# natir/br

Hardware: AMD Instinct MI355X
Metric: corrected Gbases/sec at k=19, 10 kb ONT-error reads (higher is better)
Workload: dtype u64 k-mers / 1-bit set

## Files before the change

### br_amd/csrc/brx_onelane.hip

```cpp
#include "brx_correct.hpp"

#include <stdlib.h>
#include <algorithm>
#include <vector>

using namespace brx;

namespace brx {
uint64_t scan_tmp_bytes(uint32_t n);
int exclusive_scan_lens(const uint32_t *d_lens, uint32_t n, uint64_t *d_tmp, uint64_t *d_out_offsets,
                        unsigned long long *d_total, hipStream_t s);
}


namespace {

constexpr uint32_t U_VOID = 0xffffffffu;
constexpr uint32_t U_END = 0xffffffffu;
constexpr uint32_t C_FAIL = 0xfffffff1u;
constexpr uint32_t C_VOID = 0xfffffff2u;
constexpr uint32_t U_UNWRITTEN = 0xffffffffu;
constexpr int MAX_DEPTH = 3;
constexpr uint32_t MAX_LANE_READ = 1u << 28;
#ifndef BRX_AP_EDITS
// ... 75 lines not shown
    __builtin_memcpy(&q, in + (n - 16u - j), 16);
    return make_uint4(__builtin_bswap32(q.w), __builtin_bswap32(q.z), __builtin_bswap32(q.y), __builtin_bswap32(q.x));
}
__device__ __forceinline__ uint4 ld16_raw(const uint8_t *in, uint32_t n, uint32_t j, bool flip)
{
    uint4 q;
    __builtin_memcpy(&q, in + (flip ? n - 16u - j : j), 16);
    return q;
}
__device__ __forceinline__ uint4 ld16_turn(const uint4 &q, bool flip)
{
    return flip ? make_uint4(__builtin_bswap32(q.w), __builtin_bswap32(q.z), __builtin_bswap32(q.y), __builtin_bswap32(q.x)) : q;
}
__device__ __forceinline__ uint64_t pack_start(uint64_t in_at, uint32_t r) { return (in_at >> 4) + 5ull * r; }
__device__ __forceinline__ uint64_t edit_start(uint64_t in_at, uint32_t r, uint64_t ub, uint32_t jj, uint32_t q)
{
    return (in_at >> 2) + 16ull * (ub + r + jj) + (uint64_t)(q >> 2);
}

__global__ __launch_bounds__(256) void lane_units_kernel(LaneArgs a)
{
    const uint32_t r = blockIdx.x * 256u + threadIdx.x;
    if (r >= a.p.n_reads)
        return;
    const uint8_t *in;
    uint32_t n;
    bool poisoned;
    (void)read_view(a.p, r, in, n, poisoned);
    const uint32_t C = chunk_of(a, r);
    a.nu[r] = n < 2u * C ? 1u : n / C;
}

__global__ __launch_bounds__(256) void lane_pack_kernel(LaneArgs a)
{
    for (uint32_t r = blockIdx.x; r < a.p.n_reads; r += gridDim.x) {
        const uint8_t *in;
        uint32_t n;
        bool poisoned;
        const uint64_t at = read_view(a.p, r, in, n, poisoned);
        uint32_t *dst = a.P + pack_start(at, r);
        const uint32_t ndw = (n >> 4) + 5u;
        for (uint32_t d = threadIdx.x; d < ndw; d += 256) {
            const uint32_t b = 16u * d;
            uint32_t w[4] = {0, 0, 0, 0};
            if (b + 16u <= n) {
                const uint4 q = ld16_logical(in, n, b, a.p.flip);
                w[0] = q.x;
                w[1] = q.y;
                w[2] = q.z;
                w[3] = q.w;
            } else {
                for (uint32_t t = 0; t < 16u && b + t < n; t++)
                    w[t >> 2] |= (uint32_t)ld_logical(in, n, b + t, a.p.flip) << (8u * (t & 3u));
            }
            uint32_t v = 0;
#pragma unroll
            for (int t = 0; t < 4; t++)
                v = (v << 8) | ((((w[t] >> 1) & 0x03030303u) * 0x40100401u) >> 24);
            dst[d] = v;
        }
        const uint64_t ub = a.ubase[r], ue = a.ubase[r + 1];
        for (uint64_t u = ub + threadIdx.x; u < ue; u += 256) {
            a.u_read[u] = r;
            a.u_in[u] = make_uint4((uint32_t)at, (uint32_t)(at >> 32), n, (uint32_t)(u - ub));
        }
    }
}

template <bool IDX>
__device__ __forceinline__ bool set_get(const PassParams &p, uint64_t km, int k)
{
    if (!IDX)
        return probe(p.bits, km, k);
    uint64_t key;
    const uint32_t home = index_locate(p.idx, km, k, key);
    for (uint32_t hop = 0;; hop++) {
        const int pr = index_probe_at(p.idx, key, home, hop);
        if (pr != 2)
            return pr == 1;
        if (p.bits) {
            const uint64_t h = key - 1ull;
            return (p.bits[h >> 5] >> (h & 31u)) & 1u;
        }
    }
}

template <bool IDX>
__global__ __launch_bounds__(256) void lane_mask_kernel(LaneArgs a)
{
    const PassParams &p = a.p;
    const int lane = threadIdx.x & 63;
    const int k = p.k;
    const uint64_t mask = kmask(k);
    const unsigned long long n_units = p.ctrl[CTL_LANE_UNITS];
    const unsigned long long wave = (unsigned long long)blockIdx.x * 4ull + (threadIdx.x >> 6);
    const unsigned long long n_waves = (unsigned long long)gridDim.x * 4ull;
    const bool filter = p.idx.line_bits != nullptr && p.idx.line_shift >= 6u;
    uint4 ui_next = wave < n_units ? a.u_in[wave] : make_uint4(0, 0, 0, 0);
    uint32_t r_next = wave < n_units ? a.u_read[wave] : 0u;
    for (unsigned long long u = wave; u < n_units; u += n_waves) {
        const uint4 ui = ui_next;
        const uint32_t r = r_next;
        if (u + n_waves < n_units) {
            ui_next = a.u_in[u + n_waves];
            r_next = a.u_read[u + n_waves];
        }
        const uint32_t j = ui.w, n = ui.z;
        const uint64_t at = ((uint64_t)ui.y << 32) | ui.x;
        const bool last = (uint64_t)j + 1ull == a.ubase[r + 1] - a.ubase[r];
        const uint32_t C = chunk_of(a, r);
        const uint32_t s = (j * C) & ~15u;
        const uint32_t lim = last ? n : ((j + 1u) * C) & ~15u;
        const uint32_t *row = a.P + pack_start(at, r);
        uint16_t *mrow = a.M + pack_start(at, r);
        uint64_t carry = 0;
        if (s) {
            const uint32_t b = s - 31u, w = b >> 4, sh = 2u * (b & 15u);
            const uint64_t hi = ((uint64_t)row[w] << 32) | row[w + 1];
            const uint64_t lo = row[w + 2];
            carry = (sh ? ((hi << sh) | (lo >> (32u - sh))) : hi) >> 2;
        }
        for (uint32_t e0 = s; e0 < lim; e0 += 64u) {
            const uint32_t e = e0 + (uint32_t)lane;
            const uint32_t code = (row[e >> 4] >> (30u - 2u * (e & 15u))) & 3u;
            const uint64_t km = lane_kmer64_dpp(carry, code, lane, mask);
            bool sol = false;
            if (e < lim && e + 1u >= (uint32_t)k) {
                if (IDX) {
                    uint64_t key;
                    const uint32_t home = index_locate(p.idx, km, k, key);
                    if (!filter || ((p.idx.line_bits[home >> 5] >> (home & 31u)) & 1u)) {
                        int pr = index_probe_at(p.idx, key, home, 0u);
                        for (uint32_t hop = 1; pr == 2 && !p.bits; hop++)
                            pr = index_probe_at(p.idx, key, home, hop);
                        if (pr == 2) {
                            const uint64_t h = key - 1ull;
                            pr = (p.bits[h >> 5] >> (h & 31u)) & 1u;
                        }
                        sol = pr == 1;
                    }
                } else {
                    sol = probe(p.bits, km, k);
                }
            }
            const uint64_t ball = __ballot(sol);
            if ((lane & 15) == 0 && e < lim)
                mrow[e >> 4] = (uint16_t)(ball >> lane);
            carry = ((uint64_t)(uint32_t)__builtin_amdgcn_readlane((int)(uint32_t)(km >> 32), 63) << 32) |
                    (uint32_t)__builtin_amdgcn_readlane((int)(uint32_t)km, 63);
        }
    }
}

template <bool IDX>
__global__ __launch_bounds__(256) void lane_sync_kernel(LaneArgs a)
{
    const PassParams &p = a.p;
    const uint32_t lane = threadIdx.x & 63u, half = lane >> 5, hl = lane & 31u;
    const uint32_t k = (uint32_t)p.k;
    const unsigned long long n_units = p.ctrl[CTL_LANE_UNITS];
    const unsigned long long wave = (unsigned long long)blockIdx.x * 4ull + (threadIdx.x >> 6);
    const unsigned long long n_waves = (unsigned long long)gridDim.x * 4ull;
    for (unsigned long long u0 = 2ull * wave; u0 < n_units; u0 += 2ull * n_waves) {
        const unsigned long long u = u0 + half;
        const bool mine = u < n_units;
        const uint4 ui = mine ? a.u_in[u] : make_uint4(0, 0, 0, 0);
        const uint32_t j = ui.w, n = ui.z;
        const uint32_t r = mine ? a.u_read[u] : 0u;
        const uint64_t at = ((uint64_t)ui.y << 32) | ui.x;
        const uint32_t *row = a.P + pack_start(at, r);
        const uint32_t C = chunk_of(a, r);
        const uint32_t s = j * C;
        const uint32_t lim = (s + C < n) ? s + C : n;
        const uint32_t e0 = s + k - 1u;
        bool open_ = mine && j != 0u;
        uint32_t q = (mine && j == 0u) ? 0u : U_VOID;
        uint64_t qk = 0;
        uint32_t prev32 = 0;
        for (uint32_t t = 0; __any(open_ && e0 + 32u * t < lim); t++) {
            const uint32_t e = e0 + 32u * t + hl;
            const bool valid = open_ && e < lim;
            uint64_t km = 0;
            bool sol = false;
            if (valid) {
                const uint32_t b = e + 1u - k, wd = b >> 4, sh = 2u * (b & 15u);
                const uint64_t hi = ((uint64_t)row[wd] << 32) | row[wd + 1];
                const uint64_t lo = row[wd + 2];
                km = (sh ? ((hi << sh) | (lo >> (32u - sh))) : hi) >> (64u - 2u * k);
                sol = set_get<IDX>(p, km, (int)k);
            }
            const uint64_t ball = __ballot(sol);
            const uint32_t cur32 = (uint32_t)(ball >> (32u * half));
            const uint64_t w = ((uint64_t)cur32 << 32) | prev32;
            uint64_t x = w;
            for (uint32_t rr = 1; rr < a.R; rr++)
                x &= w << rr;
            const uint32_t hit = (uint32_t)(x >> 32);
            const bool found = open_ && hit != 0u;
            const uint32_t el_l = found ? (uint32_t)__builtin_ctz(hit) : 0u;
            const uint32_t src = 32u * half + el_l;
            const uint32_t klo = (uint32_t)__shfl((int)(uint32_t)km, (int)src), khi = (uint32_t)__shfl((int)(uint32_t)(km >> 32), (int)src);
            if (found) {
                const uint32_t qq = e0 + 32u * t + el_l + 1u;
                if (qq < n) {
                    q = qq;
                    qk = ((uint64_t)khi << 32) | klo;
                }
                open_ = false;
            } else if (open_ && e0 + 32u * (t + 1u) >= lim) {
                open_ = false;
            }
            prev32 = cur32;
        }
        if (mine && hl == 0u) {
            a.u_q[u] = q;
            if (j != 0u)
                a.u_qk[u] = qk;
        }
    }
}

__global__ __launch_bounds__(256) void lane_sync_mask_kernel(LaneArgs a)
{
    const PassParams &p = a.p;
    const uint32_t k = (uint32_t)p.k;
    const unsigned long long n_units = p.ctrl[CTL_LANE_UNITS];
    for (unsigned long long u = (unsigned long long)blockIdx.x * 256ull + threadIdx.x; u < n_units; u += (unsigned long long)gridDim.x * 256ull) {
        const uint4 ui = a.u_in[u];
        const uint32_t j = ui.w, n = ui.z;
        if (j == 0) {
            a.u_q[u] = 0;
            continue;
        }
        const uint32_t r = a.u_read[u];
        const uint64_t at = ((uint64_t)ui.y << 32) | ui.x;
        const uint32_t *row = a.P + pack_start(at, r);
        const uint16_t *mrow = a.M + pack_start(at, r);
        const uint32_t C = chunk_of(a, r);
        const uint32_t s = j * C;
        const uint32_t lim = (s + C < n) ? s + C : n;
        const uint32_t e0 = s + k - 1u;
        uint32_t q = U_VOID;
        uint64_t qk = 0;
        uint64_t w = 0;
        for (uint32_t g = e0 >> 4; 16u * g < lim; g++) {
            uint32_t bits = mrow[g];
            const uint32_t base = 16u * g;
            if (base < e0)
                bits &= 0xffffu << (e0 - base);
            if (base + 16u > lim)
                bits &= 0xffffu >> (base + 16u - lim);
            w = (w >> 16) | ((uint64_t)bits << 48);
            uint64_t t = w;
            for (uint32_t rr = 1; rr < a.R; rr++)
                t &= w << rr;
            const uint32_t hit = (uint32_t)(t >> 48);
            if (hit) {
                const uint32_t el = base + (uint32_t)__builtin_ctz(hit);
                if (el + 1u < n) {
                    q = el + 1u;
                    const uint32_t b = el + 1u - k, wd = b >> 4, sh = 2u * (b & 15u);
                    const uint64_t hi = ((uint64_t)row[wd] << 32) | row[wd + 1];
                    const uint64_t lo = row[wd + 2];
                    qk = (sh ? ((hi << sh) | (lo >> (32u - sh))) : hi) >> (64u - 2u * k);
                }
                break;
            }
        }
        a.u_q[u] = q;
        a.u_qk[u] = qk;
    }
}

struct __attribute__((aligned(16))) UnitDesc {
    uint32_t n;
    uint32_t q;
    uint32_t t1;
    uint32_t tgt;
    uint64_t tgtk;
    uint64_t eat;
    uint64_t pw;
    uint32_t ecap;
    uint32_t first;
};

__global__ __launch_bounds__(256) void lane_link_kernel(LaneArgs a)
{
    const PassParams &p = a.p;
    const unsigned long long n_units = p.ctrl[CTL_LANE_UNITS];
    for (unsigned long long u = (unsigned long long)blockIdx.x * 256ull + threadIdx.x; u < n_units; u += (unsigned long long)gridDim.x * 256ull) {
        const uint32_t r = a.u_read[u];
        const uint32_t ub = (uint32_t)a.ubase[r], uend = (uint32_t)a.ubase[r + 1];
        const uint8_t *in;
        uint32_t n;
        bool poisoned;
        const uint64_t in_at = read_view(p, r, in, n, poisoned);
        UnitDesc d;
        d.n = n;
        d.q = n >= MAX_LANE_READ ? U_VOID - 1u : a.u_q[u];
        uint32_t t = (uint32_t)u + 1u;
        while (t < uend && a.u_q[t] == U_VOID)
            t++;
        const uint32_t q0 = d.q >= U_VOID - 1u ? 0u : d.q;
        d.eat = edit_start(in_at, r, ub, (uint32_t)u - ub, q0);
        uint64_t end_at;
        if (t < uend) {
            d.t1 = t;
            d.tgt = a.u_q[t];
            d.tgtk = a.u_qk[t];
            end_at = edit_start(in_at, r, ub, t - ub, d.tgt);
        } else {
            d.t1 = U_END;
            d.tgt = n;
            d.tgtk = 0;
            end_at = edit_start(in_at, r, ub, uend - ub, n);
        }
        d.ecap = (uint32_t)(end_at - d.eat);
        d.pw = pack_start(in_at, r) + (q0 >> 4);
        d.first = (uint32_t)u == ub ? 1u : 0u;
        a.u_desc[u] = d;
    }
}

enum { S_ST = 0, S_CUR = 2, S_JJ = 4, S_ACC = 8, S_PASS = 12, S_DIRTY = 16, S_SKIP = 24, S_PREV = 27, S_FIRST = 28, S_SLOW = 29 };
constexpr uint32_t MASK_STEP = 16;

template <bool IDX, int KT, bool MASK>
__global__ __launch_bounds__(256, MASK ? 6 : BRX_LANE_WAVES) void lane_kernel(LaneArgs a)
{
    const PassParams &p = a.p;
    const int k = KT ? KT : p.k;
    const uint32_t c = (uint32_t)p.c;
    const uint64_t mask = kmask(k);
    const unsigned long long n_units = p.ctrl[CTL_LANE_UNITS];
    __shared__ uint4 lc[4][256];
    const uint32_t tid = threadIdx.x;

    bool have = false, want = true;
    uint32_t u = 0, n = 0, i = 0, tgt = 0, t1 = U_END;
    uint64_t tgtk = 0;
    uint32_t depth = 0, ne = 0, ecap = 0;
// ... 1449 lines not shown
    const char *e = getenv(name);
    return e && *e ? (uint32_t)strtoul(e, nullptr, 10) : dflt;
}

void lane_ws_free(brx_chain *ch)
{
    delete (LaneWork *)ch->lane_ws;
    ch->lane_ws = nullptr;
}

int lane_pass(brx_chain *ch, const PassParams &p, const LanePassInfo &info, hipStream_t s)
{
    const bool walk = info.method != BRX_ONE;
    if (env_u32("BRX_LANE", 1u) == 0u || p.k > 31 || p.n_reads == 0)
        return BRX_ERR_UNSUPPORTED;
    if (info.method != BRX_GRAPH && (p.c < 1 || p.c > 5))
        return BRX_ERR_UNSUPPORTED;
    if (walk && env_u32("BRX_LANE_WALK", 1u) == 0u)
        return BRX_ERR_UNSUPPORTED;
    if (!walk && p.idx.lines && 32u - p.idx.line_shift > env_u32("BRX_LANE_MAX_LOG_LINES", 26u))
        return BRX_ERR_UNSUPPORTED;
    const bool idx = p.idx.lines != nullptr;
    if (!idx && !p.bits)
        return BRX_ERR_UNSUPPORTED;
    constexpr uint64_t RESIDENT = 256ull * 4ull * BRX_LANE_WAVES * 64ull;
    uint32_t C = env_u32("BRX_LANE_CHUNK", 0u);
    if (C == 0u) {
        const uint64_t want = info.in_total_bound / (4ull * RESIDENT);
        C = want < 256ull ? 256u : (want > 2048ull ? 2048u : (uint32_t)want);
    }
    if (C < 64u)
        C = 64u;
    uint32_t R = env_u32("BRX_LANE_SYNC", 4u);
    if (R < 1u)
        R = 1u;
    if (R > 32u)
        R = 32u;

    LaneWork *w = (LaneWork *)ch->lane_ws;
    if (!w) {
        w = new LaneWork();
        ch->lane_ws = w;
    }
    const bool graded = !walk && env_u32("BRX_LANE_TAIL", 0u) != 0u && p.n_reads >= 64u;
    const uint32_t r_half = graded ? p.n_reads - p.n_reads / 5u : 0xffffffffu;
    const uint32_t r_quarter = graded ? p.n_reads - p.n_reads / 20u : 0xffffffffu;
    const uint32_t c_min = graded ? ((C >> 2) < 64u ? 64u : (C >> 2)) : C;
    const uint64_t units_bound = info.in_total_bound / c_min + (uint64_t)p.n_reads + 1ull;
    if (units_bound >= 0xfffffff0ull)
        return BRX_ERR_UNSUPPORTED;
    const uint64_t p_bound = (info.in_total_bound >> 4) + 5ull * p.n_reads + 16ull;
    const uint64_t e_bound = (info.in_total_bound >> 2) + 16ull * (units_bound + 2ull * p.n_reads) + 64ull;
    const char *what = "lane pass workspace";
    const uint64_t n = p.n_reads, hr = n / 8 + 64;
    BRX_TRY(w->nu.reserve(n, hr, what));
    BRX_TRY(w->fail_list.reserve(n, hr, what));
    BRX_TRY(w->ubase.reserve(n + 1, hr, what));
    const uint64_t hu = units_bound / 8 + 64;
    BRX_TRY(w->u_read.reserve(units_bound, hu, what));
    BRX_TRY(w->u_q.reserve(units_bound, hu, what));
    BRX_TRY(w->u_qk.reserve(units_bound, hu, what));
    BRX_TRY(w->u_res.reserve(units_bound * 8, hu * 8, what));
    BRX_TRY(w->u_desc.reserve(units_bound, hu, what));
    BRX_TRY(w->u_in.reserve(units_bound, hu, what));
    BRX_TRY(w->P.reserve(p_bound, p_bound / 16, what));
    BRX_TRY(w->M.reserve(p_bound, p_bound / 16, what));
    for (int d = 0; d < MAX_DEPTH; d++)
        BRX_TRY(w->E[d].reserve(e_bound, e_bound / 16, what));
    if (walk)
        for (int d = 0; d < MAX_DEPTH; d++)
            BRX_TRY(w->BW[d].reserve(e_bound, e_bound / 16, what));
    if (scan_tmp_bytes(p.n_reads) > ch->d_scan_tmp.bytes()) {
        set_error("lane pass: scan scratch smaller than the batch");
        return BRX_ERR_ARG;
    }
    LaneArgs a;
    a.p = p;
    a.C = C;
    a.r_half = r_half;
    a.r_quarter = r_quarter;
    a.R = R;
    a.nu = w->nu;
    a.ubase = w->ubase;
    a.u_read = w->u_read;
    a.u_q = w->u_q;
    a.u_qk = w->u_qk;
    a.u_res = w->u_res;
    a.u_desc = w->u_desc;
    a.u_in = w->u_in;
    a.P = w->P;
    const uint32_t mask_mode = env_u32("BRX_LANE_MASK", 1u);
    const bool use_mask = walk ? mask_mode >= 1u : mask_mode >= 2u;
    a.M = use_mask ? w->M : nullptr;
    for (int d = 0; d < MAX_DEPTH; d++) {
        a.E[d] = w->E[d];
        a.EW[d] = reinterpret_cast<uint2 *>(w->E[d].get());
        a.BW[d] = w->BW[d];
    }
    if (info.method == BRX_GRAPH)
        a.p.c = 1;
    a.fail_list = w->fail_list;
    a.succ = nullptr;
    a.dbg = nullptr;
    DevBuf<unsigned long long> d_dbg;
#ifdef BRX_LANE_TIMING
    if (!walk && env_u32("BRX_LANE_TIMING", 0u) != 0u) {
        BRX_TRY(d_dbg.reserve(1 + 3 * 16384, 0, "lane timing"));
        BRX_HIP(hipMemsetAsync(d_dbg, 0, (1 + 3 * 16384) * 8, s));
        a.dbg = d_dbg;
    }
#endif
    if (walk && idx && env_u32("BRX_LANE_SUCC", 1u) != 0u) {
        brx_set *set = const_cast<brx_set *>(ch->set);
        std::lock_guard<std::mutex> g(set->idx_mu);
        const uint64_t n_lines = 1ull << (32u - p.idx.line_shift);
        if (!set->d_succ || set->succ_lines != n_lines || set->succ_gen != set->idx_gen) {
            if (set->succ_lines != n_lines)
                set->d_succ.reset();
            BRX_TRY(set->d_succ.reserve(n_lines, 0, "successor table"));
            set->succ_lines = n_lines;
            KernelTimer t("succ_build", s);
            const uint64_t blocks = (n_lines + 255ull) / 256ull;
            succ_build_kernel<<<(uint32_t)(blocks < 65536ull ? blocks : 65536ull), 256, 0, s>>>(p, n_lines, set->d_succ);
            BRX_HIP(hipGetLastError());
            BRX_HIP(hipStreamSynchronize(s));
            set->succ_gen = set->idx_gen;
        }
        a.succ = set->d_succ;
    }

    const uint32_t rb = (p.n_reads + 255u) / 256u;
    {
        KernelTimer t("lane_units", s);
        BRX_HIP(hipMemsetAsync(p.ctrl + CTL_LANE_UNITS, 0, (CTL_LANE_FAIL + 1 - CTL_LANE_UNITS) * 8, s));
        BRX_HIP(hipMemsetAsync(w->u_res, 0xff, units_bound * 32ull, s));
        lane_units_kernel<<<rb, 256, 0, s>>>(a);
        BRX_TRY(exclusive_scan_lens(w->nu, p.n_reads, ch->d_scan_tmp, w->ubase, p.ctrl + CTL_LANE_UNITS, s));
        const uint32_t grid = read_grid(p.n_reads, 1u << 16);
        lane_pack_kernel<<<grid, 256, 0, s>>>(a);
    }
    if (use_mask) {
        KernelTimer t("lane_mask", s);
        BRX_HIP(hipMemsetAsync(w->M, 0, p_bound * 2ull, s));
        const uint64_t waves = units_bound < 256ull * 32ull ? units_bound : 256ull * 32ull;
        const uint32_t blocks = (uint32_t)((waves + 3) / 4);
        if (idx)
            lane_mask_kernel<true><<<blocks, 256, 0, s>>>(a);
        else
            lane_mask_kernel<false><<<blocks, 256, 0, s>>>(a);
    }
    {
        KernelTimer t("lane_sync", s);
        const uint64_t waves = units_bound < 256ull * 32ull ? units_bound : 256ull * 32ull;
        const uint32_t blocks = (uint32_t)((waves + 3) / 4);
        if (use_mask) {
            const uint64_t ub = (units_bound + 255ull) / 256ull;
            lane_sync_mask_kernel<<<(uint32_t)(ub < 16384ull ? ub : 16384ull), 256, 0, s>>>(a);
        } else if (idx)
            lane_sync_kernel<true><<<blocks, 256, 0, s>>>(a);
        else
            lane_sync_kernel<false><<<blocks, 256, 0, s>>>(a);
        const uint64_t lb = (units_bound + 255ull) / 256ull;
        lane_link_kernel<<<(uint32_t)(lb < 4096ull ? lb : 4096ull), 256, 0, s>>>(a);
    }
    {
        static const char *names[5] = {"correct_pass", "correct_pass_two", "correct_pass_graph", "correct_pass_greedy", "correct_pass_gap_size"};
        KernelTimer t(names[info.method], s);
        const uint64_t want = (units_bound + 255ull) / 256ull;
        const uint64_t waves = walk ? (uint64_t)walk_waves(info.method) : (use_mask ? 6ull : (uint64_t)BRX_LANE_WAVES);
        const uint32_t blocks = (uint32_t)(want < 256ull * waves ? want : 256ull * waves);
        if (info.method == BRX_ONE) {
            if (idx && use_mask)
                launch_lane<true, true>(a, blocks, s);
            else if (idx)
                launch_lane<true, false>(a, blocks, s);
            else if (use_mask)
                launch_lane<false, true>(a, blocks, s);
            else
                launch_lane<false, false>(a, blocks, s);
        } else if (info.method == BRX_GRAPH) {
            if (idx)
                launch_lane_walk<true, BRX_GRAPH>(a, blocks, s);
            else
                launch_lane_walk<false, BRX_GRAPH>(a, blocks, s);
        } else {
            if (idx)
                launch_lane_walk<true, BRX_GAP_SIZE>(a, blocks, s);
            else
                launch_lane_walk<false, BRX_GAP_SIZE>(a, blocks, s);
        }
    }
    if (d_dbg) {
        std::vector<unsigned long long> h(1 + 3 * 16384);
        BRX_HIP(hipMemcpyAsync(h.data(), d_dbg, h.size() * 8, hipMemcpyDeviceToHost, s));
        BRX_HIP(hipStreamSynchronize(s));
        const size_t nw = (size_t)(h[0] < 16384ull ? h[0] : 16384ull);
        if (nw) {
            std::vector<double> st(nw), en(nw), it(nw), lr(nw);
            unsigned long long t0 = ~0ull;
            for (size_t i = 0; i < nw; i++)
                t0 = h[1 + 3 * i] < t0 ? h[1 + 3 * i] : t0;
            for (size_t i = 0; i < nw; i++) {
                st[i] = (double)(h[1 + 3 * i] - t0) * 0.01;
                en[i] = (double)(h[2 + 3 * i] - t0) * 0.01;
                it[i] = (double)(h[3 + 3 * i] & 0xffffffffull);
                lr[i] = (double)(h[3 + 3 * i] >> 32);
            }
            auto pct = [](std::vector<double> v, double q) { std::sort(v.begin(), v.end()); return v[(size_t)(q * (double)(v.size() - 1))]; };
            fprintf(stderr, "[lane timing] %zu waves, %u reads; start us p0/p50/p100 %.0f/%.0f/%.0f; end us p0/p10/p50/p90/p99/p100 %.0f/%.0f/%.0f/%.0f/%.0f/%.0f; "
                            "loop iterations per wave p0/p50/p100 %.0f/%.0f/%.0f; lane-rounds per wave p50/p100 %.0f/%.0f\n",
                    nw, p.n_reads, pct(st, 0), pct(st, .5), pct(st, 1), pct(en, 0), pct(en, .1), pct(en, .5), pct(en, .9), pct(en, .99), pct(en, 1),
                    pct(it, 0), pct(it, .5), pct(it, 1), pct(lr, .5), pct(lr, 1));
        }
    }
    {
        KernelTimer t("lane_apply", s);
        const uint32_t gcap = env_u32("BRX_AP_GRID", 1u << 20);
        const uint32_t grid = p.n_reads < gcap ? p.n_reads : gcap;
        if (walk)
            lane_apply_walk_kernel<<<grid, 256, 0, s>>>(a);
        else
            lane_apply_kernel<<<grid, AP_BS, 0, s>>>(a);
    }
    {
        KernelTimer t("lane_redo", s);
        PassParams q = p;
        q.only = w->fail_list;
        q.only_n = p.ctrl + CTL_LANE_FAIL;
        BRX_HIP(hipMemsetAsync(p.ctrl + CTL_WORK, 0, 8, s));
        if (walk)
            BRX_TRY(launch_walk_list(q, info.method, s));
        else
            BRX_TRY(launch_one_list(q, s));
    }
    BRX_HIP(hipGetLastError());
    return BRX_OK;
}

}
```

### br_amd/csrc/brx_index.hip

```cpp
#include "brx_internal.hpp"
#include "brx_index.hpp"

#include <stdlib.h>

using namespace brx;

namespace {

template <bool CHAIN>
__global__ __launch_bounds__(256) void index_insert_kernel(const uint64_t *__restrict__ keys, uint64_t n, uint64_t *__restrict__ lines,
                                                           uint32_t line_shift, uint32_t m, uint32_t w, int k,
                                                           unsigned long long *__restrict__ n_overflow, uint32_t *__restrict__ line_bits)
{
    const uint64_t stride = (uint64_t)gridDim.x * blockDim.x;
    const uint32_t line_mask = 0xffffffffu >> line_shift;
    uint32_t lost = 0;
    for (uint64_t i = (uint64_t)blockIdx.x * blockDim.x + threadIdx.x; i < n; i += stride) {
        const uint64_t h = keys[i];
        const uint64_t canon = (h << 1) | (uint64_t)(popc64(h) & 1);
        const uint64_t rc = revcomp(canon, k);
        uint32_t line = index_line_of(minimizer_of(canon, rc, m, w), line_shift);
        bool counted = false;
        for (uint32_t walked = 0; walked <= line_mask; walked++) {
            unsigned long long *L = reinterpret_cast<unsigned long long *>(lines) + (uint64_t)line * 8ull;
            const unsigned long long seen = __hip_atomic_load(L + 7, __ATOMIC_RELAXED, __HIP_MEMORY_SCOPE_AGENT);
            uint32_t slot = IDX_SLOTS;
            if ((uint32_t)seen < (uint32_t)IDX_SLOTS)
                slot = (uint32_t)atomicAdd(L + 7, 1ull);
            if (slot < (uint32_t)IDX_SLOTS) {
                L[slot] = h + 1ull;
                if (slot == 0u)
                    atomicOr(line_bits + (line >> 5), 1u << (line & 31u));
                break;
            }
            {
                const unsigned long long want = (unsigned long long)IDX_OVERFLOW | (counted ? 0ull : (unsigned long long)idx_sig_bit(h + 1ull));
                if ((seen & want) != want)
                    atomicOr(L + 7, want);
            }
            if (!counted) {
                lost++;
                counted = true;
            }
            if (!CHAIN)
                break;
            line = (line + 1u) & line_mask;
        }
    }
    for (int d = 32; d > 0; d >>= 1)
        lost += __shfl_down(lost, d);
    if ((threadIdx.x & 63) == 0 && lost)
        atomicAdd(n_overflow, (unsigned long long)lost);
}

__global__ void index_get_kernel(IdxView v, const uint32_t *__restrict__ bits, const uint64_t *__restrict__ kmers, uint32_t n, int k,
                                 uint8_t *__restrict__ out, unsigned long long *__restrict__ n_fallback)
{
    const uint32_t i = blockIdx.x * blockDim.x + threadIdx.x;
    if (i >= n)
        return;
    const uint64_t fwd = kmers[i] & kmask(k);
    int r = index_probe(v, fwd, k);
    if (r == 2) {
        atomicAdd(n_fallback, 1ull);
        if (bits) {
            const uint64_t h = khash(fwd, k);
            r = (bits[h >> 5] >> (h & 31u)) & 1u;
        } else {
            for (uint32_t hop = 1; r == 2; hop++)
                r = index_probe(v, fwd, k, hop);
        }
    }
    out[i] = (uint8_t)r;
}

__global__ __launch_bounds__(256) void table_rehash_kernel(const uint64_t *__restrict__ old_lines, uint64_t n_old_lines, int k,
                                                           uint64_t *__restrict__ lines, uint32_t line_shift, uint32_t m, uint32_t w)
{
    const uint64_t stride = (uint64_t)gridDim.x * blockDim.x;
    for (uint64_t i = (uint64_t)blockIdx.x * blockDim.x + threadIdx.x; i < n_old_lines * IDX_SLOTS; i += stride) {
        const uint64_t v = old_lines[(i / IDX_SLOTS) * 8ull + (i % IDX_SLOTS)];
        if (v) {
            const uint64_t h = v - 1ull;
            (void)table_find_or_insert(lines, line_shift, m, w, k, (h << 1) | (uint64_t)(popc64(h) & 1));
        }
    }
}

__global__ __launch_bounds__(256) void table_to_bits_kernel(const uint64_t *__restrict__ lines, uint64_t n_lines, uint32_t *__restrict__ bits,
                                                            uint64_t nbits)
{
    const uint64_t stride = (uint64_t)gridDim.x * blockDim.x;
    for (uint64_t i = (uint64_t)blockIdx.x * blockDim.x + threadIdx.x; i < n_lines * IDX_SLOTS; i += stride) {
        const uint64_t v = lines[(i / IDX_SLOTS) * 8ull + (i % IDX_SLOTS)];
        if (v && v - 1ull < nbits)
            atomicOr(bits + ((v - 1ull) >> 5), 1u << ((v - 1ull) & 31u));
    }
}

__global__ void keys_to_bits_kernel(const uint64_t *__restrict__ keys, const unsigned long long *__restrict__ n_ptr, uint32_t *__restrict__ bits,
                                    uint64_t nbits)
{
    const uint64_t n = *n_ptr;
    const uint64_t stride = (uint64_t)gridDim.x * blockDim.x;
    for (uint64_t i = (uint64_t)blockIdx.x * blockDim.x + threadIdx.x; i < n; i += stride) {
        const uint64_t h = keys[i];
        if (h < nbits)
            atomicOr(bits + (h >> 5), 1u << (h & 31u));
    }
}

int env_int(const char *name, int dflt)
{
    const char *e = getenv(name);
    return (e && *e) ? atoi(e) : dflt;
}

}

namespace brx {

bool index_wanted(int k)
{
    if (sparse_k(k))
        return true;

    return (k & 1) && k >= env_int("BRX_INDEX_MIN_K", 15) && k >= 5 && env_int("BRX_INDEX", 1) != 0;
}

int index_auto_m(int k, uint64_t n_keys)
{
    int m = 3;
    while (m < IDX_AUTO_MAX_M && (1ull << (2 * m - 1)) < 16ull * n_keys)
        m += 2;
    if (m == IDX_AUTO_MAX_M && (1ull << (2 * IDX_AUTO_MAX_M - 1)) < 16ull * n_keys && k - IDX_MAX_M + 1 >= 3)
        return IDX_MAX_M;
    if (m > k - 2)
        m = k - 2;
    if (!(m & 1))
        m--;
    return m < 3 ? 3 : m;
}

static int index_build_locked(brx_set *set, const uint64_t *d_keys, uint64_t n, int m, int log_lines, hipStream_t s)
{
    const int k = set->k;
    if (!(k & 1) || k < 5 || k > 31) {
        set_error("probe index needs odd 5 <= k <= 31 (k=%d)", k);
        return BRX_ERR_UNSUPPORTED;
    }
    BRX_TRY(use_device(set->device));
    if (m <= 0)
        m = env_int("BRX_INDEX_M", 0);
    if (m <= 0)
        m = index_auto_m(k, n);
    if ((!(m & 1) && m != 16) || m < 3 || m > IDX_MAX_M || k - m + 1 < 2) {
        set_error("probe index: minimizer length %d must be odd (or 16), 3..%d and shorter than the %d-mer", m, IDX_MAX_M, k);
        return BRX_ERR_ARG;
    }
    if (log_lines <= 0)
        log_lines = env_int("BRX_INDEX_LOG_LINES", 0);
    if (log_lines <= 0) {
        log_lines = 10;
        while (log_lines < 29 && (1ull << log_lines) < n + n / 2)
            log_lines++;
    }
    while (no_bits(set) && log_lines < 30 && (7ull << log_lines) < n + n / 4)
        log_lines++;
    if (log_lines < 4 || log_lines > 30) {
        set_error("probe index: log2(lines)=%d out of range 4..30", log_lines);
        return BRX_ERR_ARG;
    }
    if (no_bits(set) && (7ull << log_lines) < n + n / 4) {
        set_error("set without bit vector: %llu solid k-mers do not fit a chained table of 2^%d lines (7 slots each)",
                  (unsigned long long)n, log_lines);
        return BRX_ERR_NOMEM;
    }
    set->idx_valid = false;
    set->idx_gen++;
    const uint64_t n_lines = 1ull << log_lines;
    if (set->lines_alloc < n_lines) {
        set->d_lines.reset();
        set->lines_alloc = 0;
        BRX_TRY(set->d_lines.reserve_bytes(n_lines * 64ull + n_lines / 8ull + 64ull, 0, "probe index"));
        set->lines_alloc = n_lines;
    }
    DevBuf<unsigned long long> d_ovf;
    BRX_TRY(d_ovf.reserve(1, 0, "probe index build"));
    BRX_HIP(hipMemsetAsync(d_ovf, 0, 8, s));
    {
        KernelTimer t("index_zero", s);
        BRX_HIP(hipMemsetAsync(set->d_lines, 0, n_lines * 64ull + n_lines / 8ull + 64ull, s));
    }
    if (n) {
        KernelTimer t("index_insert", s);
        uint64_t blocks = (n + 255) / 256;
        if (blocks > 256 * 16)
            blocks = 256 * 16;
        if (no_bits(set))
            index_insert_kernel<true><<<(int)blocks, 256, 0, s>>>(d_keys, n, set->d_lines, 32u - (uint32_t)log_lines, (uint32_t)m,
                                                                  (uint32_t)(k - m + 1), k, d_ovf, (uint32_t *)(set->d_lines + n_lines * 8ull));
        else
            index_insert_kernel<false><<<(int)blocks, 256, 0, s>>>(d_keys, n, set->d_lines, 32u - (uint32_t)log_lines, (uint32_t)m,
                                                                   (uint32_t)(k - m + 1), k, d_ovf, (uint32_t *)(set->d_lines + n_lines * 8ull));
        BRX_HIP(hipGetLastError());
    }
    unsigned long long ovf = 0;
    BRX_HIP(hipMemcpyAsync(&ovf, d_ovf, 8, hipMemcpyDeviceToHost, s));
    BRX_HIP(hipStreamSynchronize(s));
    set->idx_log_lines = (uint32_t)log_lines;
    set->idx_m = (uint32_t)m;
    set->idx_keys = n;
    set->idx_overflow_keys = ovf;
    set->idx_exact = no_bits(set);
    set->idx_open = false;
    set->idx_linebits = true;
    set->idx_valid = true;
    set->idx_gen++;
    return BRX_OK;
}

int index_build_from_keys(brx_set *set, const uint64_t *d_keys, uint64_t n, int m, int log_lines, hipStream_t s)
{
    std::lock_guard<std::mutex> g(set->idx_mu);
    return index_build_locked(set, d_keys, n, m, log_lines, s);
}

int index_insert_reads(brx_set *set, const uint8_t *d_bases, const uint64_t *d_offsets, uint32_t n_reads, uint64_t total_bases,
                       hipStream_t s)
{
    const int k = set->k;
    if (!set->sparse || !(k & 1) || k < 5 || k > 31) {
        set_error("k-mer insertion into a sparse set needs an odd 5 <= k <= 31 (k=%d%s)", k, set->sparse ? "" : ", set is not sparse");
        return BRX_ERR_UNSUPPORTED;
    }
    BRX_TRY(use_device(set->device));
    std::lock_guard<std::mutex> g(set->idx_mu);
    if (set->idx_valid && !set->idx_open) {
        set_error("the set was built by counting; k-mers cannot be added to it");
        return BRX_ERR_UNSUPPORTED;
    }
    if (!set->idx_valid) {
        set->idx_keys = 0;
        set->idx_overflow_keys = 0;
    }
    const uint64_t need = set->idx_keys + total_bases;
    const bool have = set->idx_valid && set->d_lines;
    if (!have || (7ull << set->idx_log_lines) < 2ull * need) {
        int log_lines = 12;
        while (log_lines < 30 && (7ull << log_lines) < 3ull * need)
            log_lines++;
        if ((7ull << log_lines) < need + need / 4) {
            set_error("sparse set: %llu k-mers do not fit the largest table", (unsigned long long)need);
            return BRX_ERR_NOMEM;
        }
        int m = env_int("BRX_INDEX_M", 0);
        if (m <= 0)
            m = index_auto_m(k, need);
        if ((!(m & 1) && m != 16) || m < 3 || m > IDX_MAX_M || m > k - 1) {
            set_error("probe index: bad minimizer length %d for k=%d", m, k);
            return BRX_ERR_ARG;
        }
        DevBuf<uint64_t> nl;
        BRX_TRY(nl.reserve_bytes((64ull << log_lines) + ((1ull << log_lines) >> 3) + 64ull, 0, "sparse set table"));
        BRX_HIP(hipMemsetAsync(nl, 0, 64ull << log_lines, s));
        if (have && set->idx_keys) {
            KernelTimer t("index_rehash", s);
            table_rehash_kernel<<<256 * 8, 256, 0, s>>>(set->d_lines, 1ull << set->idx_log_lines, k, nl, 32u - (uint32_t)log_lines,
                                                        (uint32_t)m, (uint32_t)(k - m + 1));
        }
        BRX_HIP(hipStreamSynchronize(s));
        set->d_lines = std::move(nl);
        set->lines_alloc = 1ull << log_lines;
        set->idx_log_lines = (uint32_t)log_lines;
        set->idx_m = (uint32_t)m;
    }
    DevBuf<unsigned long long> d_new;
    BRX_TRY(d_new.reserve(1, 0, "sparse set insert"));
    BRX_HIP(hipMemsetAsync(d_new, 0, 8, s));
    if (n_reads) {
        KernelTimer t("index_insert_reads", s);
        BRX_TRY(flat_presence_insert(d_bases, d_offsets, n_reads, total_bases, k, nullptr, set->d_lines, 32u - set->idx_log_lines,
                                     set->idx_m, d_new, s));
    }
    unsigned long long added = 0;
    BRX_HIP(hipMemcpyAsync(&added, d_new, 8, hipMemcpyDeviceToHost, s));
    BRX_HIP(hipStreamSynchronize(s));
    set->idx_keys += added;
    set->idx_exact = true;
    set->idx_linebits = false;
    set->idx_open = true;
    set->idx_valid = true;
    set->idx_gen++;
    set->keylist_valid = false;
    return BRX_OK;
}

int ensure_bits(const brx_set *cset, hipStream_t s, const char *what)
{
    brx_set *set = const_cast<brx_set *>(cset);
    if (set->sparse) {
        set_error("%s needs the bit vector; a sparse set (k=%d) has none", what, set->k);
        return BRX_ERR_UNSUPPORTED;
    }
    if (!set->bits_stale)
        return BRX_OK;
    BRX_TRY(use_device(set->device));
    std::lock_guard<std::mutex> g(set->idx_mu);
    if (!set->bits_stale)
        return BRX_OK;
    KernelTimer t("bits_materialise", s);
    BRX_HIP(hipMemsetAsync(set->d_bits, 0, set->nwords * 4, s));
    if (set->keylist_valid) {
        keys_to_bits_kernel<<<256 * 8, 256, 0, s>>>(set->d_keylist, set->d_keylist_n, set->d_bits, set->nwords * 32);
    } else if (set->idx_valid && set->idx_exact) {
        table_to_bits_kernel<<<256 * 16, 256, 0, s>>>(set->d_lines, 1ull << set->idx_log_lines, set->d_bits, set->nwords * 32);
    } else {
        set_error("%s: the set has neither bits, key list nor an exact index", what);
        return BRX_ERR_ARG;
    }
    BRX_HIP(hipGetLastError());
    BRX_HIP(hipStreamSynchronize(s));
    set->bits_stale = false;
    return BRX_OK;
}

int index_ensure(const brx_set *cset, hipStream_t s)
{
    brx_set *set = const_cast<brx_set *>(cset);
    if (!index_wanted(set->k) && !no_bits(set))
        return BRX_OK;
    std::lock_guard<std::mutex> g(set->idx_mu);
    if (set->idx_valid || set->idx_declined)
        return BRX_OK;
    BRX_TRY(use_device(set->device));
    uint64_t n = 0;
    bool listed = false;
    if (set->keylist_valid) {
        unsigned long long nl = 0;
        BRX_HIP(hipMemcpyAsync(&nl, set->d_keylist_n, 8, hipMemcpyDeviceToHost, s));
        BRX_HIP(hipStreamSynchronize(s));
        listed = nl <= set->d_keylist.cap();
        n = nl;
    }
    if (!listed) {
        BRX_HIP(hipStreamSynchronize(s));
        BRX_TRY(brx_set_popcount(set, &n));
    }
    if (no_bits(set) && !listed) {
        set_error("set without bit vector and without a complete key list (%llu solid k-mers counted, room for %llu)", (unsigned long long)n,
                  (unsigned long long)set->d_keylist.cap());
        return BRX_ERR_NOMEM;
    }
    if (!no_bits(set) && set->k - index_auto_m(set->k, n) + 1 < 3 && env_int("BRX_INDEX_M", 0) <= 0) {
        set->idx_declined = true;
        return BRX_OK;
    }
    if (listed)
        return index_build_locked(set, set->d_keylist, n, 0, 0, s);
    DevBuf<uint64_t> d_keys;
    BRX_TRY(d_keys.reserve(n ? n : 1, 0, "keys of the set"));
    uint64_t got = 0;
    BRX_TRY(brx_set_extract_keys_device(set, 0, set->nwords * 32, d_keys, n, &got, s));
    return index_build_locked(set, d_keys, got, 0, 0, s);
}

// ... 201 lines not shown
```

Baseline: 27.65.

## Software-pipeline unit descriptor and first packed-row loads in lane_sync_kernel

The lane_sync kernel now prefetches unit descriptors three iterations ahead and the first packed k-mer words two iterations ahead, so the first window of each unit uses preloaded data rather than issuing dependent global loads. The aim is to hide the latency of the chain descriptor → pack_start → row load behind the work on the current unit. It also adds an environment-variable cap on the sync grid size, which defaults high enough to leave the grid unchanged. In exchange it uses more registers per thread and issues extra loads for units past the end.

```diff
diff --git a/br_amd/csrc/brx_onelane.hip b/br_amd/csrc/brx_onelane.hip
--- a/br_amd/csrc/brx_onelane.hip
+++ b/br_amd/csrc/brx_onelane.hip
@@ -251,6 +251,45 @@
     }
 }
 
+
+struct SyncUnit {
+    uint4 ui;
+    uint32_t r;
+    bool mine;
+};
+__device__ __forceinline__ SyncUnit sync_unit_load(const LaneArgs &a, unsigned long long u, unsigned long long n_units)
+{
+    SyncUnit x;
+    x.mine = u < n_units;
+    x.ui = x.mine ? a.u_in[u] : make_uint4(0, 0, 0, 0);
+    x.r = x.mine ? a.u_read[u] : 0u;
+    return x;
+}
+__device__ __forceinline__ bool sync_first_base(const LaneArgs &a, const SyncUnit &x, uint32_t k, uint32_t hl, uint32_t &b)
+{
+    const uint32_t j = x.ui.w, n = x.ui.z;
+    const uint32_t C = chunk_of(a, x.r);
+    const uint32_t s = j * C;
+    const uint32_t lim = (s + C < n) ? s + C : n;
+    b = s + hl;
+    return x.mine && j != 0u && b + k - 1u < lim;
+}
+__device__ __forceinline__ uint3 sync_first_rows(const LaneArgs &a, const SyncUnit &x, uint32_t k, uint32_t hl)
+{
+    uint32_t b;
+    if (!sync_first_base(a, x, k, hl, b))
+        return make_uint3(0, 0, 0);
+    const uint64_t at = ((uint64_t)x.ui.y << 32) | x.ui.x;
+    const uint32_t *row = a.P + pack_start(at, x.r) + (b >> 4);
+    return make_uint3(row[0], row[1], row[2]);
+}
+__device__ __forceinline__ uint64_t sync_cut(const uint3 &dw, uint32_t b, uint32_t k)
+{
+    const uint32_t sh = 2u * (b & 15u);
+    const uint64_t hi = ((uint64_t)dw.x << 32) | dw.y;
+    const uint64_t lo = dw.z;
+    return (sh ? ((hi << sh) | (lo >> (32u - sh))) : hi) >> (64u - 2u * k);
+}
 template <bool IDX>
 __global__ __launch_bounds__(256) void lane_sync_kernel(LaneArgs a)
 {
@@ -259,13 +298,25 @@
     const uint32_t k = (uint32_t)p.k;
     const unsigned long long n_units = p.ctrl[CTL_LANE_UNITS];
     const unsigned long long wave = (unsigned long long)blockIdx.x * 4ull + (threadIdx.x >> 6);
-    const unsigned long long n_waves = (unsigned long long)gridDim.x * 4ull;
-    for (unsigned long long u0 = 2ull * wave; u0 < n_units; u0 += 2ull * n_waves) {
+    const unsigned long long step = 2ull * (unsigned long long)gridDim.x * 4ull;
+    SyncUnit x1 = sync_unit_load(a, 2ull * wave + half, n_units);
+    SyncUnit x2 = sync_unit_load(a, 2ull * wave + step + half, n_units);
+    SyncUnit x3 = sync_unit_load(a, 2ull * wave + 2ull * step + half, n_units);
+    uint3 d1 = sync_first_rows(a, x1, k, hl);
+    uint3 d2 = sync_first_rows(a, x2, k, hl);
+    for (unsigned long long u0 = 2ull * wave; u0 < n_units; u0 += step) {
         const unsigned long long u = u0 + half;
-        const bool mine = u < n_units;
-        const uint4 ui = mine ? a.u_in[u] : make_uint4(0, 0, 0, 0);
+        const SyncUnit cu = x1;
+        const uint3 d = d1;
+        x1 = x2;
+        x2 = x3;
+        x3 = sync_unit_load(a, u + 3ull * step, n_units);
+        d1 = d2;
+        d2 = sync_first_rows(a, x2, k, hl);
+        const bool mine = cu.mine;
+        const uint4 ui = cu.ui;
         const uint32_t j = ui.w, n = ui.z;
-        const uint32_t r = mine ? a.u_read[u] : 0u;
+        const uint32_t r = cu.r;
         const uint64_t at = ((uint64_t)ui.y << 32) | ui.x;
         const uint32_t *row = a.P + pack_start(at, r);
         const uint32_t C = chunk_of(a, r);
@@ -282,10 +333,11 @@
             uint64_t km = 0;
             bool sol = false;
             if (valid) {
-                const uint32_t b = e + 1u - k, wd = b >> 4, sh = 2u * (b & 15u);
-                const uint64_t hi = ((uint64_t)row[wd] << 32) | row[wd + 1];
-                const uint64_t lo = row[wd + 2];
-                km = (sh ? ((hi << sh) | (lo >> (32u - sh))) : hi) >> (64u - 2u * k);
+                const uint32_t b = e + 1u - k, wd = b >> 4;
+                uint3 dw = d;
+                if (t != 0u)
+                    dw = make_uint3(row[wd], row[wd + 1], row[wd + 2]);
+                km = sync_cut(dw, b, k);
                 sol = set_get<IDX>(p, km, (int)k);
             }
             const uint64_t ball = __ballot(sol);
@@ -2041,7 +2093,9 @@
     {
         KernelTimer t("lane_sync", s);
         const uint64_t waves = units_bound < 256ull * 32ull ? units_bound : 256ull * 32ull;
-        const uint32_t blocks = (uint32_t)((waves + 3) / 4);
+        const uint32_t scap = env_u32("BRX_LANE_SYNC_GRID", 1u << 20);
+        const uint32_t sblocks = (uint32_t)((waves + 3) / 4);
+        const uint32_t blocks = sblocks < scap ? sblocks : (scap ? scap : 1u);
         if (use_mask) {
             const uint64_t ub = (units_bound + 255ull) / 256ull;
             lane_sync_mask_kernel<<<(uint32_t)(ub < 16384ull ? ub : 16384ull), 256, 0, s>>>(a);
```

Measured after the change: 27.37. 0.99x the previous value.

## Build probe index by sorting keys into line regions and filling them in LDS

Applied to the files above, without the earlier changes.

Replaces the global-atomic scatter insert with a region-based build. Keys are radix-sorted by their home line's region, each workgroup builds a region's lines in LDS with workgroup-scope atomics, and the image is streamed out with nontemporal stores, which also removes the separate zeroing memset. Keys that chain past a region's end go to a continuation list that the old global kernel handles afterwards, and the old path remains as a fallback. This adds a sort pass, scratch allocation and a host sync, and changes line placement order relative to the old insert.

```diff
diff --git a/br_amd/csrc/brx_index.hip b/br_amd/csrc/brx_index.hip
--- a/br_amd/csrc/brx_index.hip
+++ b/br_amd/csrc/brx_index.hip
@@ -1,26 +1,37 @@
 #include "brx_internal.hpp"
 #include "brx_index.hpp"
 
+#include <stdio.h>
 #include <stdlib.h>
 
+#include <rocprim/device/device_radix_sort.hpp>
+
 using namespace brx;
 
 namespace {
+
+__device__ __forceinline__ uint32_t key_home_line(uint64_t h, uint32_t line_shift, uint32_t m, uint32_t w, int k)
+{
+    const uint64_t canon = (h << 1) | (uint64_t)(popc64(h) & 1);
+    return index_line_of(minimizer_of(canon, revcomp(canon, k), m, w), line_shift);
+}
 
 template <bool CHAIN>
 __global__ __launch_bounds__(256) void index_insert_kernel(const uint64_t *__restrict__ keys, uint64_t n, uint64_t *__restrict__ lines,
                                                            uint32_t line_shift, uint32_t m, uint32_t w, int k,
-                                                           unsigned long long *__restrict__ n_overflow, uint32_t *__restrict__ line_bits)
+                                                           unsigned long long *__restrict__ n_overflow, uint32_t *__restrict__ line_bits,
+                                                           const uint32_t *__restrict__ cont_lines = nullptr,
+                                                           const unsigned long long *__restrict__ n_dev = nullptr)
 {
     const uint64_t stride = (uint64_t)gridDim.x * blockDim.x;
     const uint32_t line_mask = 0xffffffffu >> line_shift;
     uint32_t lost = 0;
+    if (n_dev && *n_dev < n)
+        n = *n_dev;
     for (uint64_t i = (uint64_t)blockIdx.x * blockDim.x + threadIdx.x; i < n; i += stride) {
         const uint64_t h = keys[i];
-        const uint64_t canon = (h << 1) | (uint64_t)(popc64(h) & 1);
-        const uint64_t rc = revcomp(canon, k);
-        uint32_t line = index_line_of(minimizer_of(canon, rc, m, w), line_shift);
-        bool counted = false;
+        uint32_t line = cont_lines ? cont_lines[i] : key_home_line(h, line_shift, m, w, k);
+        bool counted = cont_lines != nullptr;
         for (uint32_t walked = 0; walked <= line_mask; walked++) {
             unsigned long long *L = reinterpret_cast<unsigned long long *>(lines) + (uint64_t)line * 8ull;
             const unsigned long long seen = __hip_atomic_load(L + 7, __ATOMIC_RELAXED, __HIP_MEMORY_SCOPE_AGENT);
@@ -53,6 +64,144 @@
         atomicAdd(n_overflow, (unsigned long long)lost);
 }
 
+#ifndef BRX_INDEX_REGION_LOG
+#define BRX_INDEX_REGION_LOG 10
+#endif
+#ifndef BRX_INDEX_LINES_THREADS
+#define BRX_INDEX_LINES_THREADS 512
+#endif
+#ifndef BRX_INDEX_ORDER_PAIRS
+#define BRX_INDEX_ORDER_PAIRS 0
+#endif
+#ifndef BRX_INDEX_NT_STORE
+#define BRX_INDEX_NT_STORE 1
+#endif
+constexpr uint32_t IDX_REGION_LOG = BRX_INDEX_REGION_LOG;
+constexpr uint32_t IDX_LINES_THREADS = BRX_INDEX_LINES_THREADS;
+static_assert(IDX_REGION_LOG >= 6 && IDX_REGION_LOG <= 11, "a region's image must fit the LDS of a CU");
+static_assert(IDX_LINES_THREADS % 64 == 0 && IDX_LINES_THREADS <= 1024, "whole waves");
+
+__global__ __launch_bounds__(256) void index_region_of_kernel(const uint64_t *__restrict__ keys, uint32_t n, uint32_t line_shift, uint32_t m,
+                                                              uint32_t w, int k, uint32_t region_log, uint32_t *__restrict__ region_of,
+                                                              uint64_t *__restrict__ packed, uint32_t key_bits)
+{
+    const uint32_t stride = gridDim.x * blockDim.x;
+    for (uint32_t i = blockIdx.x * blockDim.x + threadIdx.x; i < n; i += stride) {
+        const uint64_t h = keys[i];
+        const uint32_t region = key_home_line(h, line_shift, m, w, k) >> region_log;
+        if (packed)
+            packed[i] = ((uint64_t)region << key_bits) | (h & ((1ull << key_bits) - 1ull));
+        else
+            region_of[i] = region;
+    }
+}
+
+__global__ __launch_bounds__(256) void index_region_first_kernel(const uint32_t *__restrict__ sorted, const uint64_t *__restrict__ packed,
+                                                                 uint32_t key_bits, uint32_t n, uint32_t n_regions,
+                                                                 uint32_t *__restrict__ first)
+{
+    const uint64_t stride = (uint64_t)gridDim.x * blockDim.x;
+    auto region_at = [&](uint64_t i) { return packed ? (uint32_t)(packed[i] >> key_bits) : (sorted ? sorted[i] : 0u); };
+    for (uint64_t i = (uint64_t)blockIdx.x * blockDim.x + threadIdx.x; i <= n; i += stride) {
+        const uint32_t lo = i == 0 ? 0u : region_at(i - 1) + 1u;
+        uint32_t hi = i == n ? n_regions : region_at(i);
+        if (hi > n_regions)
+            hi = n_regions;
+        for (uint32_t r = lo; r <= hi; r++)
+            first[r] = (uint32_t)i;
+    }
+}
+
+template <bool CHAIN>
+__global__ __launch_bounds__(IDX_LINES_THREADS) void index_lines_kernel(const uint64_t *__restrict__ keys, uint64_t key_mask,
+                                                                        const uint32_t *__restrict__ first, uint32_t n_regions, uint32_t region_log, uint64_t *__restrict__ lines,
+                                                                        uint32_t line_shift, uint32_t m, uint32_t w, int k,
+                                                                        unsigned long long *__restrict__ n_overflow,
+                                                                        uint32_t *__restrict__ line_bits, uint64_t *__restrict__ cont_keys,
+                                                                        uint32_t *__restrict__ cont_lines, unsigned long long *__restrict__ n_cont,
+                                                                        uint64_t cont_cap)
+{
+    extern __shared__ __attribute__((aligned(16))) unsigned long long img[];
+    const uint32_t rlines = 1u << region_log;
+    const uint32_t line_mask = 0xffffffffu >> line_shift;
+    uint4 *img4 = reinterpret_cast<uint4 *>(img);
+    uint32_t lost = 0;
+    for (uint32_t r = blockIdx.x; r < n_regions; r += gridDim.x) {
+        for (uint32_t i = threadIdx.x; i < rlines * 4u; i += IDX_LINES_THREADS)
+            img4[i] = make_uint4(0u, 0u, 0u, 0u);
+        __syncthreads();
+        const uint32_t base = r << region_log;
+        const uint32_t end = first[r + 1];
+        for (uint32_t i = first[r] + threadIdx.x; i < end; i += IDX_LINES_THREADS) {
+            const uint64_t h = keys[i] & key_mask;
+            uint32_t ll = (key_home_line(h, line_shift, m, w, k) - base) & (rlines - 1u);
+            bool counted = false;
+            for (;;) {
+                unsigned long long *L = img + ll * 8u;
+                const unsigned long long seen = __hip_atomic_load(L + 7, __ATOMIC_RELAXED, __HIP_MEMORY_SCOPE_WORKGROUP);
+                uint32_t slot = IDX_SLOTS;
+                if ((uint32_t)seen < (uint32_t)IDX_SLOTS)
+                    slot = (uint32_t)__hip_atomic_fetch_add(L + 7, 1ull, __ATOMIC_RELAXED, __HIP_MEMORY_SCOPE_WORKGROUP);
+                if (slot < (uint32_t)IDX_SLOTS) {
+                    L[slot] = h + 1ull;
+                    break;
+                }
+                {
+                    const unsigned long long want = (unsigned long long)IDX_OVERFLOW | (counted ? 0ull : (unsigned long long)idx_sig_bit(h + 1ull));
+                    if ((seen & want) != want)
+                        (void)__hip_atomic_fetch_or(L + 7, want, __ATOMIC_RELAXED, __HIP_MEMORY_SCOPE_WORKGROUP);
+                }
+                if (!counted) {
+                    lost++;
+                    counted = true;
+                }
+                if (!CHAIN)
+                    break;
+                if (++ll == rlines) {
+                    const unsigned long long at = atomicAdd(n_cont, 1ull);
+                    if (at < cont_cap) {
+                        cont_keys[at] = h;
+                        cont_lines[at] = (base + rlines) & line_mask;
+                    }
+                    break;
+                }
+            }
+        }
+        __syncthreads();
+        uint4 *out = reinterpret_cast<uint4 *>(lines + (uint64_t)base * 8ull);
+        for (uint32_t i = threadIdx.x; i < rlines * 4u; i += IDX_LINES_THREADS) {
+#if BRX_INDEX_NT_STORE
+            typedef uint32_t u32x4 __attribute__((ext_vector_type(4)));
+            __builtin_nontemporal_store(reinterpret_cast<const u32x4 *>(img4)[i], reinterpret_cast<u32x4 *>(out) + i);
+#else
+            out[i] = img4[i];
+#endif
+        }
+        if (rlines >= 64u) {
+            for (uint32_t l = threadIdx.x; l < rlines; l += IDX_LINES_THREADS) {
+                const unsigned long long b = __ballot((uint32_t)img[l * 8u + 7u] != 0u);
+                if ((threadIdx.x & 63u) == 0u)
+                    reinterpret_cast<unsigned long long *>(line_bits)[(base + l) >> 6] = b;
+            }
+        } else if (threadIdx.x < 64u) {
+            const unsigned long long b = __ballot(threadIdx.x < rlines && (uint32_t)img[(threadIdx.x & (rlines - 1u)) * 8u + 7u] != 0u);
+            if (threadIdx.x == 0u) {
+                if (rlines == 32u)
+                    line_bits[0] = (uint32_t)b;
+                else
+                    reinterpret_cast<uint16_t *>(line_bits)[0] = (uint16_t)b;
+            }
+        }
+        if (r == n_regions - 1u && threadIdx.x < 64u)
+            reinterpret_cast<uint8_t *>(line_bits)[(((uint64_t)line_mask + 1ull) >> 3) + threadIdx.x] = 0;
+        __syncthreads();
+    }
+    for (int d = 32; d > 0; d >>= 1)
+        lost += __shfl_down(lost, d);
+    if ((threadIdx.x & 63) == 0 && lost)
+        atomicAdd(n_overflow, (unsigned long long)lost);
+}
+
 __global__ void index_get_kernel(IdxView v, const uint32_t *__restrict__ bits, const uint64_t *__restrict__ kmers, uint32_t n, int k,
                                  uint8_t *__restrict__ out, unsigned long long *__restrict__ n_fallback)
 {
@@ -142,6 +291,97 @@
     return m < 3 ? 3 : m;
 }
 
+static int index_build_regions(const uint64_t *d_keys, uint64_t n, uint64_t *d_lines, int log_lines, uint32_t m, uint32_t w, int k, bool chain,
+                               unsigned long long *d_counts, hipStream_t s, DevBuf<uint8_t> &scratch, bool &done, uint64_t &cont_cap)
+{
+    done = false;
+    if (n >= (1ull << 31))
+        return BRX_OK;
+    const uint32_t line_shift = 32u - (uint32_t)log_lines;
+    const uint32_t region_log = (uint32_t)log_lines < IDX_REGION_LOG ? (uint32_t)log_lines : IDX_REGION_LOG;
+    const uint32_t sort_bits = (uint32_t)log_lines - region_log;
+    const uint32_t n_regions = 1u << sort_bits;
+    const uint64_t n_lines = 1ull << log_lines;
+    cont_cap = chain ? n / 8ull + 4096ull : 0ull;
+
+    const bool ordered = sort_bits && n;
+    const uint32_t key_bits = 2u * (uint32_t)k - 1u;
+    const bool pack = ordered && key_bits + sort_bits <= 64u && !BRX_INDEX_ORDER_PAIRS;
+    size_t sort_bytes = 0;
+    if (pack)
+        BRX_HIP(rocprim::radix_sort_keys(nullptr, sort_bytes, (const uint64_t *)nullptr, (uint64_t *)nullptr, (uint32_t)n, key_bits,
+                                         key_bits + sort_bits, s));
+    else if (ordered)
+        BRX_HIP(rocprim::radix_sort_pairs(nullptr, sort_bytes, (const uint32_t *)nullptr, (uint32_t *)nullptr, d_keys, (uint64_t *)nullptr,
+                                          (uint32_t)n, 0u, sort_bits, s));
+    auto up = [](uint64_t b) { return (b + 255ull) & ~255ull; };
+    const uint64_t o_first = 0, o_ckeys = o_first + up(((uint64_t)n_regions + 1ull) * 4ull), o_clines = o_ckeys + up(cont_cap * 8ull),
+                   o_sorted = o_clines + up(cont_cap * 4ull), o_rin = o_sorted + up(ordered ? n * 8ull : 0ull),
+                   o_rout = o_rin + up(!ordered ? 0ull : pack ? n * 8ull : n * 4ull), o_tmp = o_rout + up(ordered && !pack ? n * 4ull : 0ull),
+                   total = o_tmp + up(sort_bytes);
+    {
+        const uint64_t pad = (uint64_t)env_int("BRX_INDEX_SCRATCH_PAD_GB", 0) << 30;
+        void *p = nullptr;
+        if (dev_alloc(&p, total + pad) != hipSuccess) {
+            (void)hipGetLastError();
+            return BRX_OK;
+        }
+        scratch.adopt((uint8_t *)p, total + pad);
+    }
+    uint32_t *const first = (uint32_t *)(scratch + o_first);
+    uint64_t *const cont_keys = (uint64_t *)(scratch + o_ckeys);
+    uint32_t *const cont_lines = (uint32_t *)(scratch + o_clines);
+    uint64_t *const sorted = (uint64_t *)(scratch + o_sorted);
+    uint32_t *const rin = (uint32_t *)(scratch + o_rin), *const rout = (uint32_t *)(scratch + o_rout);
+    uint32_t *const line_bits = (uint32_t *)(d_lines + n_lines * 8ull);
+    {
+        KernelTimer t("index_sort", s);
+        if (ordered) {
+            uint32_t blocks = (uint32_t)((n + 255) / 256);
+            index_region_of_kernel<<<blocks > 4096u ? 4096u : blocks, 256, 0, s>>>(d_keys, (uint32_t)n, line_shift, m, w, k, region_log, rin,
+                                                                                   pack ? (uint64_t *)rin : nullptr, key_bits);
+            BRX_HIP(hipGetLastError());
+            if (pack)
+                BRX_HIP(rocprim::radix_sort_keys(scratch + o_tmp, sort_bytes, (const uint64_t *)rin, sorted, (uint32_t)n, key_bits,
+                                                 key_bits + sort_bits, s));
+            else
+                BRX_HIP(rocprim::radix_sort_pairs(scratch + o_tmp, sort_bytes, (const uint32_t *)rin, rout, d_keys, sorted, (uint32_t)n, 0u,
+                                                  sort_bits, s));
+        }
+        uint32_t blocks = (uint32_t)((n + 256) / 256);
+        index_region_first_kernel<<<blocks > 4096u ? 4096u : blocks, 256, 0, s>>>(ordered && !pack ? rout : nullptr, pack ? sorted : nullptr,
+                                                                                  key_bits, (uint32_t)n, n_regions, first);
+        BRX_HIP(hipGetLastError());
+    }
+    {
+        KernelTimer t("index_lines", s);
+        const uint32_t lds = 64u << region_log;
+        const uint32_t grid = n_regions < 2048u ? n_regions : 2048u;
+        const uint64_t *const in = ordered ? sorted : d_keys;
+        const uint64_t key_mask = pack ? (1ull << key_bits) - 1ull : ~0ull;
+        if (lds > 65536u) {
+            BRX_HIP(hipFuncSetAttribute((const void *)index_lines_kernel<true>, hipFuncAttributeMaxDynamicSharedMemorySize, (int)lds));
+            BRX_HIP(hipFuncSetAttribute((const void *)index_lines_kernel<false>, hipFuncAttributeMaxDynamicSharedMemorySize, (int)lds));
+        }
+        if (chain)
+            index_lines_kernel<true><<<grid, IDX_LINES_THREADS, lds, s>>>(in, key_mask, first, n_regions, region_log, d_lines, line_shift, m, w, k, d_counts,
+                                                                         line_bits, cont_keys, cont_lines, d_counts + 1, cont_cap);
+        else
+            index_lines_kernel<false><<<grid, IDX_LINES_THREADS, lds, s>>>(in, key_mask, first, n_regions, region_log, d_lines, line_shift, m, w, k, d_counts,
+                                                                          line_bits, nullptr, nullptr, d_counts + 1, 0);
+        BRX_HIP(hipGetLastError());
+    }
+    if (chain && n) {
+        KernelTimer t("index_insert", s);
+        const uint64_t blocks = (cont_cap + 255) / 256;
+        index_insert_kernel<true><<<(int)(blocks > 1024 ? 1024 : blocks), 256, 0, s>>>(cont_keys, cont_cap, d_lines, line_shift, m, w, k, d_counts,
+                                                                                       line_bits, cont_lines, d_counts + 1);
+        BRX_HIP(hipGetLastError());
+    }
+    done = true;
+    return BRX_OK;
+}
+
 static int index_build_locked(brx_set *set, const uint64_t *d_keys, uint64_t n, int m, int log_lines, hipStream_t s)
 {
     const int k = set->k;
@@ -186,32 +426,56 @@
         set->lines_alloc = n_lines;
     }
     DevBuf<unsigned long long> d_ovf;
-    BRX_TRY(d_ovf.reserve(1, 0, "probe index build"));
-    BRX_HIP(hipMemsetAsync(d_ovf, 0, 8, s));
-    {
-        KernelTimer t("index_zero", s);
-        BRX_HIP(hipMemsetAsync(set->d_lines, 0, n_lines * 64ull + n_lines / 8ull + 64ull, s));
-    }
-    if (n) {
-        KernelTimer t("index_insert", s);
-        uint64_t blocks = (n + 255) / 256;
-        if (blocks > 256 * 16)
-            blocks = 256 * 16;
-        if (no_bits(set))
-            index_insert_kernel<true><<<(int)blocks, 256, 0, s>>>(d_keys, n, set->d_lines, 32u - (uint32_t)log_lines, (uint32_t)m,
-                                                                  (uint32_t)(k - m + 1), k, d_ovf, (uint32_t *)(set->d_lines + n_lines * 8ull));
-        else
-            index_insert_kernel<false><<<(int)blocks, 256, 0, s>>>(d_keys, n, set->d_lines, 32u - (uint32_t)log_lines, (uint32_t)m,
-                                                                   (uint32_t)(k - m + 1), k, d_ovf, (uint32_t *)(set->d_lines + n_lines * 8ull));
-        BRX_HIP(hipGetLastError());
-    }
-    unsigned long long ovf = 0;
-    BRX_HIP(hipMemcpyAsync(&ovf, d_ovf, 8, hipMemcpyDeviceToHost, s));
-    BRX_HIP(hipStreamSynchronize(s));
+    BRX_TRY(d_ovf.reserve(2, 0, "probe index build"));
+    BRX_HIP(hipMemsetAsync(d_ovf, 0, 16, s));
+    uint32_t *const line_bits = (uint32_t *)(set->d_lines + n_lines * 8ull);
+    const uint32_t line_shift = 32u - (uint32_t)log_lines, w = (uint32_t)(k - m + 1);
+    unsigned long long ovf[2] = {0, 0};
+    bool by_regions = false;
+    uint64_t cont_cap = 0;
+    DevBuf<uint8_t> scratch;
+    const bool want_regions = env_int("BRX_INDEX_BUILD", 1) != 0;
+    if (want_regions) {
+        const int st = index_build_regions(d_keys, n, set->d_lines, log_lines, (uint32_t)m, w, k, no_bits(set), d_ovf, s, scratch, by_regions, cont_cap);
+        if (st != BRX_OK) {
+            (void)hipStreamSynchronize(s);
+            return st;
+        }
+    }
+    if (by_regions) {
+        BRX_HIP(hipMemcpyAsync(ovf, d_ovf, 16, hipMemcpyDeviceToHost, s));
+        BRX_HIP(hipStreamSynchronize(s));
+        if (ovf[1] > cont_cap) {
+            by_regions = false;
+            BRX_HIP(hipMemsetAsync(d_ovf, 0, 16, s));
+        } else if (env_int("BRX_INDEX_TRACE", 0)) {
+            fprintf(stderr, "brx index build: 2^%d lines, %llu keys, %llu turned away by their home line, %llu left their region\n",
+                    log_lines, (unsigned long long)n, ovf[0], ovf[1]);
+        }
+    }
+    if (!by_regions) {
+        {
+            KernelTimer t("index_zero", s);
+            BRX_HIP(hipMemsetAsync(set->d_lines, 0, n_lines * 64ull + n_lines / 8ull + 64ull, s));
+        }
+        if (n) {
+            KernelTimer t("index_insert", s);
+            uint64_t blocks = (n + 255) / 256;
+            if (blocks > 256 * 16)
+                blocks = 256 * 16;
+            if (no_bits(set))
+                index_insert_kernel<true><<<(int)blocks, 256, 0, s>>>(d_keys, n, set->d_lines, line_shift, (uint32_t)m, w, k, d_ovf, line_bits);
+            else
+                index_insert_kernel<false><<<(int)blocks, 256, 0, s>>>(d_keys, n, set->d_lines, line_shift, (uint32_t)m, w, k, d_ovf, line_bits);
+            BRX_HIP(hipGetLastError());
+        }
+        BRX_HIP(hipMemcpyAsync(ovf, d_ovf, 8, hipMemcpyDeviceToHost, s));
+        BRX_HIP(hipStreamSynchronize(s));
+    }
     set->idx_log_lines = (uint32_t)log_lines;
     set->idx_m = (uint32_t)m;
     set->idx_keys = n;
-    set->idx_overflow_keys = ovf;
+    set->idx_overflow_keys = ovf[0];
     set->idx_exact = no_bits(set);
     set->idx_open = false;
     set->idx_linebits = true;
```

Measured after the change: 27.08 before, 27.66 after, median of 6. +2.1%, better.
